# leggedrobotics/rayen

Measured on AMD Instinct MI355X. Metric: feasible projections/sec at k=64, 128 lin+4 quad+2 SOC; max violation, higher is better.
Workload: dtype f32

## Files before the change

rayen_amd/csrc/rayen_mfma_pair_wl.hip:

```cpp
#include "rayen_split_image.h"

#include <algorithm>
#include <cstdlib>
#include <mutex>
#include <type_traits>

namespace rayen {

namespace {
#ifndef RAYEN_WL_WAVES
#define RAYEN_WL_WAVES 16
#endif
#ifndef RAYEN_WL_NT
#define RAYEN_WL_NT 1
#endif
#ifndef RAYEN_WL_AHEAD
#define RAYEN_WL_AHEAD 0
#endif
constexpr int kWlWaves = RAYEN_WL_WAVES;
constexpr int kWlNT = RAYEN_WL_NT;
#ifndef RAYEN_WL_ABL
#define RAYEN_WL_ABL 0
#endif
#ifndef RAYEN_WL_HEAD
#define RAYEN_WL_HEAD 1
#endif
#ifndef RAYEN_WL_AUXR2
#define RAYEN_WL_AUXR2 16
#endif
template <int NKK, bool MAPPED = false> struct WlGeom { static constexpr int AUXR = NKK == 2 ? (MAPPED ? 8 : RAYEN_WL_AUXR2) : 32; };
#ifndef RAYEN_WL_SR
#define RAYEN_WL_SR 0
#endif
constexpr int wl_stage_rows(int nt) { return RAYEN_WL_SR ? RAYEN_WL_SR : (nt == 1 ? 16 : 32); }
constexpr int wl_region_bytes(int nkk, int nt) {
  return nt * (nkk == 2 ? WlGeom<2>::AUXR : WlGeom<1>::AUXR) * 128 > wl_stage_rows(nt) * 128 ? nt * (nkk == 2 ? WlGeom<2>::AUXR : WlGeom<1>::AUXR) * 128
                                                                                             : wl_stage_rows(nt) * 128;
}
__device__ __forceinline__ void wl_dma16(const char* gbase, const unsigned voff, const unsigned lds) {
  unsigned keep;
  uint64_t asm_base;
  asm volatile(RAYEN_ASM_BASE_COPY "s_mov_b32 %[k], m0\n\ts_mov_b32 m0, %[lds]\n\ts_nop 0\n\tglobal_load_lds_dwordx4 %[off], " RAYEN_ASM_BASE "\n\ts_mov_b32 m0, %[k]"
               : [k] "=&s"(keep), [b] "=&s"(asm_base)
               : [off] "v"(voff), [base] "s"(gbase), [lds] "s"(lds)
               : "memory");
}
#ifndef RAYEN_WL_SWAP
#define RAYEN_WL_SWAP 1
#endif
template <bool SWAP> __device__ __forceinline__ float wl_half_sum(const float x) {
  if constexpr (SWAP && RAYEN_WL_SWAP) {
    const unsigned u = __builtin_bit_cast(unsigned, x);
    const auto r = __builtin_amdgcn_permlane32_swap(u, u, false, false);
    return __builtin_bit_cast(float, (unsigned)r[0]) + __builtin_bit_cast(float, (unsigned)r[1]);
  } else {
    return x + xhalf(x);
  }
}
template <bool SWAP> __device__ __forceinline__ float wl_half_max(const float x) {
  if constexpr (SWAP && RAYEN_WL_SWAP) {
    const unsigned u = __builtin_bit_cast(unsigned, x);
    const auto r = __builtin_amdgcn_permlane32_swap(u, u, false, false);
    return fmaxf(__builtin_bit_cast(float, (unsigned)r[0]), __builtin_bit_cast(float, (unsigned)r[1]));
  } else {
    return fmaxf(x, xhalf(x));
  }
}
#ifndef RAYEN_WL_NANNV2
#define RAYEN_WL_NANNV2 1
#endif
__device__ __forceinline__ void wl_set_level(const int level) {
  if (level <= 0) __builtin_amdgcn_s_setprio(3);
  else if (level == 1) __builtin_amdgcn_s_setprio(2);
  else if (level == 2) __builtin_amdgcn_s_setprio(1);
  else __builtin_amdgcn_s_setprio(0);
}
constexpr int kWlStageRowsMapped = 8;
constexpr int wl_region_bytes_mapped(int nkk, int nt) {
  return nt * (nkk == 2 ? WlGeom<2, true>::AUXR : WlGeom<1, true>::AUXR) * 128 > kWlStageRowsMapped * 128
             ? nt * (nkk == 2 ? WlGeom<2, true>::AUXR : WlGeom<1, true>::AUXR) * 128
             : kWlStageRowsMapped * 128;
}
}

#ifdef RAYEN_WL_STAMPS
#ifndef RAYEN_WL_STAMP_ROUND
#define RAYEN_WL_STAMP_ROUND 1
#endif
__device__ unsigned long long wl_stamp_buf[2 * 40 * 4];
extern "C" int rayen_debug_wl_stamps(void* dst, size_t bytes) {
  return hipMemcpyFromSymbol(dst, HIP_SYMBOL(wl_stamp_buf), bytes < sizeof(wl_stamp_buf) ? bytes : sizeof(wl_stamp_buf)) == hipSuccess ? 0 : -1;
}
#define RAYEN_WL_STAMP(item, slot)                                                                              \
  do {                                                                                                          \
    if (stamp_on && lane == 0 && (item) < 40) wl_stamp_buf[((wave >> 2) * 40 + (item)) * 4 + (slot)] = __builtin_amdgcn_s_memtime(); \
  } while (0)
#else
#define RAYEN_WL_STAMP(item, slot) do { } while (0)
#endif
#ifdef RAYEN_WL_CLOCK
constexpr int kWlClockSlots = 10;
__device__ unsigned long long wl_clock_buf[16 * 16 * kWlClockSlots];
extern "C" int rayen_debug_wl_clock(void* dst, size_t bytes) {
  return hipMemcpyFromSymbol(dst, HIP_SYMBOL(wl_clock_buf), bytes < sizeof(wl_clock_buf) ? bytes : sizeof(wl_clock_buf)) == hipSuccess ? 0 : -1;
}
#define RAYEN_WL_CLOCK_AT(slot)                                               \
  do {                                                                        \
    if (probe) {                                                              \
      clock_at[2 * (slot) + 0] = __builtin_amdgcn_s_memtime();                \
      clock_at[2 * (slot) + 1] = __builtin_amdgcn_s_memrealtime();            \
    }                                                                         \
  } while (0)
#else
#define RAYEN_WL_CLOCK_AT(slot) do { } while (0)
#endif

template <int NKK, bool TRACK, int NT, int NW, int NKX = 0, bool SCREEN = false, bool DRAIN = false>
__global__ __launch_bounds__(NW * 64, 1) void mfma_pair_wl_kernel(
    const f16x8* __restrict__ Wh, const MItem* __restrict__ items, int n_items,
    const MPack* __restrict__ packs, const float* __restrict__ y0, int n_tiles, int n,
    const float* __restrict__ v, int64_t B, int64_t ldv, float* __restrict__ y, int64_t ldy,
    float* __restrict__ kappa_out, int32_t* __restrict__ active_out,
    int32_t* __restrict__ nan_flag, const float w_scale, const float w_inv,
    const f16x8* __restrict__ mimg, int n_in, float* __restrict__ v_out, int64_t ldvo,
    const WlScreen* __restrict__ scr, unsigned* __restrict__ scr_count, const int probe_on) {
  static_assert(!SCREEN || (NT == 1 && NKX == 0), "screening: one sample tile per wave, no mapper in front");
  static_assert(!DRAIN || NKX == 0, "progress-ordered priority: the instances without a mapper");
  constexpr int NS = NKK * 2, NCH = NS * 2, NQ = NKK * 4, AUXR = WlGeom<NKK, (NKX > 0)>::AUXR;
  constexpr int NSX = NKX * 2, NQX = NKX * 4, MCH = NKK * NSX * 2;
  constexpr bool SWAP = NKX == 0;
  constexpr bool NANNV2 = SCREEN && RAYEN_WL_NANNV2 != 0;
  extern __shared__ __attribute__((aligned(1024))) char wl_smem[];
  const int lane = threadIdx.x & 63;
  const int wave = __builtin_amdgcn_readfirstlane(threadIdx.x >> 6);
  const int col = lane & 31;
  const int hi = lane >> 5;
  char* const wimg = wl_smem;
  constexpr int REGION = NKX > 0 ? wl_region_bytes_mapped(NKK, NT) : wl_region_bytes(NKK, NT);
  constexpr int SR = NKX > 0 ? kWlStageRowsMapped : wl_stage_rows(NT);
  char* const mlds = wl_smem + (size_t)n_tiles * (NCH * 1024);
  char* const stage = mlds + MCH * 1024 + wave * REGION;
  float (*const aux_lds)[AUXR][32] = reinterpret_cast<float (*)[AUXR][32]>(stage);
  float* const y0_lds = reinterpret_cast<float*>(mlds + MCH * 1024 + NW * REGION);
  float* const bias_lds = y0_lds + NKK * 32;
  unsigned* const take_lds = reinterpret_cast<unsigned*>(bias_lds + (NKX > 0 ? NKK * 32 : 0));
  const int64_t n_groups = (B + NT * 32 - 1) / (NT * 32);
  const int64_t grp_stride = (int64_t)gridDim.x;
  int64_t grp = (int64_t)blockIdx.x + (int64_t)wave * grp_stride;
  bool bad = false;
  bool first_walk = true;
  unsigned skipped = 0;
#ifdef RAYEN_WL_STAMPS
  int stamp_round = 0;
  bool stamp_on = false;
#endif
#ifdef RAYEN_WL_CLOCK
  const bool probe = (blockIdx.x & 15) == 0 && (blockIdx.x >> 4) < 16;
  unsigned long long clock_at[8] = {0, 0, 0, 0, 0, 0, 0, 0};
  int clock_groups = 0;
  RAYEN_WL_CLOCK_AT(0);
#endif
  [[maybe_unused]] int drain_level = 0, drain_at = 0x7FFFFFFF;

  for (int i = threadIdx.x; i < NKK * 32; i += NW * 64) y0_lds[i] = y0[i];
  if (threadIdx.x == 0) *take_lds = NW;
  float gm_inv = 1.f;
  int gm_exp = 0;
  if constexpr (NKX > 0) {
    const float* tail = reinterpret_cast<const float*>(mimg + (size_t)MCH * 64);
    const float gm = tail[NKK * 32];
    gm_inv = tail[NKK * 32 + 1];
    gm_exp = (int)((__builtin_bit_cast(unsigned, gm) >> 23) & 255u) - 127;
    for (int i = threadIdx.x; i < NKK * 32; i += NW * 64) bias_lds[i] = tail[i] * gm;
  }
#if !(RAYEN_WL_HEAD & 1)
  {
    const int n_chunks = n_tiles * NCH;
    const char* src = reinterpret_cast<const char*>(Wh) + lane * 16;
#pragma unroll 4
    for (int c = wave; c < n_chunks; c += NW)
      *reinterpret_cast<u32x4*>(wimg + c * 1024 + lane * 16) = *reinterpret_cast<const u32x4*>(src + (size_t)c * 1024);
  }
#endif

  const __amdgpu_buffer_rsrc_t v_rsrc =
      __builtin_amdgcn_make_buffer_rsrc(const_cast<float*>(v), 0, (int)(unsigned)((uint64_t)B * (uint64_t)ldv * 4u), 0x00020000);
  const __amdgpu_buffer_rsrc_t y_rsrc =
      __builtin_amdgcn_make_buffer_rsrc(y, 0, (int)(unsigned)((uint64_t)B * (uint64_t)ldy * 4u), 0x00020000);
  const unsigned v_lane_off = (unsigned)col * (unsigned)ldv * 4u + 16u * (unsigned)hi;
  const unsigned y_lane_off = (unsigned)(lane >> 3) * (unsigned)ldy * 4u + 16u * (unsigned)((lane & 7) ^ ((lane >> 3) & 7));
  f32x4 vraw[NT][NQ];
  f32x4 xraw[NT][NKX > 0 ? NQX : 1];
  const bool ragged_n = n < NKK * 32;
  const bool ragged_in = NKX > 0 && n_in < NKX * 32;
  constexpr unsigned kNowhere = 0xFFFFFFF0u;
  auto request = [&](const int64_t g) {
    const unsigned goff = v_lane_off + (unsigned)g * (unsigned)(NT * 32) * (unsigned)ldv * 4u;
#pragma unroll
    for (int t = 0; t < NT; ++t) {
      if constexpr (NKX > 0) {
        if (__builtin_expect(ragged_in, 0)) {
          asm volatile("; ragged width" ::: "memory");
#pragma unroll
          for (int q = 0; q < NQX; ++q) {
            unsigned off = goff + (unsigned)t * 32u * (unsigned)ldv * 4u + 32u * q;
            off = (8 * q + 4 * hi < n_in) ? off : kNowhere;
            xraw[t][q] = __builtin_bit_cast(f32x4, __builtin_amdgcn_raw_buffer_load_b128(v_rsrc, off, 0, 0));
          }
        } else {
#pragma unroll
          for (int q = 0; q < NQX; ++q)
            xraw[t][q] = __builtin_bit_cast(f32x4, __builtin_amdgcn_raw_buffer_load_b128(
                v_rsrc, goff + (unsigned)t * 32u * (unsigned)ldv * 4u + 32u * q, 0, 0));
        }
      } else {
        if (__builtin_expect(ragged_n, 0)) {
          asm volatile("; ragged width" ::: "memory");
#pragma unroll
          for (int q = 0; q < NQ; ++q) {
            unsigned off = goff + (unsigned)t * 32u * (unsigned)ldv * 4u + 32u * q;
            off = (8 * q + 4 * hi < n) ? off : kNowhere;
            vraw[t][q] = __builtin_bit_cast(f32x4, __builtin_amdgcn_raw_buffer_load_b128(v_rsrc, off, 0, 0));
          }
        } else {
#pragma unroll
          for (int q = 0; q < NQ; ++q)
            vraw[t][q] = __builtin_bit_cast(f32x4, __builtin_amdgcn_raw_buffer_load_b128(
                v_rsrc, goff + (unsigned)t * 32u * (unsigned)ldv * 4u + 32u * q, 0, 0));
        }
      }
    }
  };
  float m_half[NT];
  auto half_max = [&]() {
#pragma unroll
    for (int t = 0; t < NT; ++t) {
      float m = 0.f;
      if constexpr (NKX > 0) {
#pragma unroll
        for (int q = 0; q < NQX; ++q)
#pragma unroll
          for (int c = 0; c < 4; ++c) m = fmaxf(m, __builtin_fabsf(xraw[t][q][c]));
      } else {
#pragma unroll
        for (int q = 0; q < NQ; ++q)
#pragma unroll
          for (int c = 0; c < 4; ++c) m = fmaxf(m, __builtin_fabsf(vraw[t][q][c]));
      }
      m_half[t] = m;
      asm volatile("" : "+v"(m_half[t]));
    }
  };
#pragma unroll
  for (int t = 0; t < NT; ++t) m_half[t] = 0.f;
  auto put_lines = [&](const f32x4 (&o)[4], const int h, const int t, const __amdgpu_buffer_rsrc_t rsrc, const unsigned goff,
                       const unsigned ld4, const int width, const bool ragged) {
#pragma unroll
    for (int part = 0; part < 32 / SR; ++part) {
      if (SR == 32 || (col / SR) == part) {
        char* slot = stage + (col % SR) * 128;
#pragma unroll
        for (int qq = 0; qq < 4; ++qq) *reinterpret_cast<f32x4*>(slot + (((2 * qq + hi) ^ (col & 7)) * 16)) = o[qq];
      }
      __builtin_amdgcn_wave_barrier();
#pragma unroll
      for (int i = 0; i < SR / 8; ++i) {
        const int r = 8 * i + (lane >> 3);
        const f32x4 x = *reinterpret_cast<const f32x4*>(stage + r * 128 + (lane & 7) * 16);
        unsigned off = goff + (unsigned)(t * 32 + part * SR + 8 * i) * ld4 + 128u * h;
        if (__builtin_expect(ragged, 0)) {
          asm volatile("; ragged width" ::: "memory");
          off = (32 * h + 4 * ((lane & 7) ^ ((lane >> 3) & 7)) < width) ? off : kNowhere;
        }
        if constexpr (RAYEN_WL_ABL & 2) { if (x[0] == 123.456f) __builtin_amdgcn_raw_buffer_store_b128(__builtin_bit_cast(u32x4, x), rsrc, off, 0, 0); }
        else if constexpr (RAYEN_WL_ABL & 8) __builtin_amdgcn_raw_buffer_store_b128(__builtin_bit_cast(u32x4, x), rsrc, off, 0, 0);
        else __builtin_amdgcn_raw_buffer_store_b128(__builtin_bit_cast(u32x4, x), rsrc, off, 0, 2);
      }
      __builtin_amdgcn_wave_barrier();
    }
  };
#if RAYEN_WL_HEAD
  {
    const int n_chunks = n_tiles * NCH;
    const unsigned img_at = __builtin_amdgcn_readfirstlane((unsigned)reinterpret_cast<uintptr_t>(wimg));
    const unsigned lane16 = lane * 16;
    if (RAYEN_WL_HEAD & 1)
      for (int c = wave; c < n_chunks; c += NW)
        wl_dma16(reinterpret_cast<const char*>(Wh) + (size_t)c * 1024, lane16, img_at + c * 1024);
    if constexpr (NKX > 0)
      for (int c = wave; c < MCH; c += NW)
        wl_dma16(reinterpret_cast<const char*>(mimg) + (size_t)c * 1024, lane16, img_at + (n_chunks + c) * 1024);
    if ((RAYEN_WL_HEAD & 2) && (grp + 1) * (NT * 32) <= B) {
      const char* gb = reinterpret_cast<const char*>(v + grp * (NT * 32) * ldv);
      const unsigned lds_at = __builtin_amdgcn_readfirstlane((unsigned)reinterpret_cast<uintptr_t>(stage));
#pragma unroll
      for (int t = 0; t < NT; ++t)
#pragma unroll
        for (int q = 0; q < NQ; ++q) wl_dma16(gb, v_lane_off + (unsigned)t * 32u * (unsigned)ldv * 4u + 32u * q, lds_at);
      asm volatile("s_waitcnt vmcnt(%0)" : : "n"(NT * NQ) : "memory");
    } else {
      asm volatile("s_waitcnt vmcnt(0)" ::: "memory");
    }
  }
#endif
  if (RAYEN_WL_AHEAD && grp < n_groups) {
    request(grp);
    half_max();
  }
  __syncthreads();

  while (grp < n_groups) {
    const int64_t s_base = grp * (NT * 32);
    int taken = 0;
    if (lane == 0) taken = (int)atomicAdd(take_lds, 1u);
    const int64_t next = (int64_t)blockIdx.x + (int64_t)__builtin_amdgcn_readfirstlane(taken) * grp_stride;
    bool live[NT];
#pragma unroll
    for (int t = 0; t < NT; ++t) live[t] = (s_base + t * 32 + col) < B;
    if constexpr (DRAIN) {
      wl_set_level(drain_level);
      drain_level = drain_level < 3 ? drain_level + 1 : 3;
      drain_at = next >= n_groups ? n_items / 3 : 0x7FFFFFFF;
    }
    if constexpr (!RAYEN_WL_AHEAD) {
      request(grp);
      half_max();
    }

#ifdef RAYEN_WL_STAMPS
    stamp_on = blockIdx.x == 0 && (wave == 0 || wave == 4) && stamp_round == RAYEN_WL_STAMP_ROUND;
    ++stamp_round;
    RAYEN_WL_STAMP(38, 0);
#endif
    f16x8 vb[NT][2][NS];
    float v_scl[NT], v_inv[NT];
    bool nan_row[NT];
    int sx_exp[NT];
    if constexpr (NKX > 0) {
      static_assert(NT == 1, "the mapped instances walk one sample tile per wave");
      static_assert((RAYEN_WL_HEAD & 1) != 0, "the mapper's image is copied by the LDS-DMA head");
      const unsigned vo_goff = (unsigned)(lane >> 3) * (unsigned)ldvo * 4u + 16u * (unsigned)((lane & 7) ^ ((lane >> 3) & 7)) +
                               (unsigned)s_base * (unsigned)ldvo * 4u;
      const __amdgpu_buffer_rsrc_t vo_rsrc =
          __builtin_amdgcn_make_buffer_rsrc(v_out, 0, (int)(unsigned)((uint64_t)B * (uint64_t)ldvo * 4u), 0x00020000);
#pragma unroll
      for (int t = 0; t < NT; ++t) {
        const float mx = fmaxf(m_half[t], xhalf(m_half[t]));
        float sx, sx_inv;
        pow2_scale(mx, sx, sx_inv, sx_exp[t]);
        f32x16 macc[NKK];
#pragma unroll
        for (int tp = 0; tp < NKK; ++tp)
#pragma unroll
          for (int a4 = 0; a4 < 4; ++a4) {
            const f32x4 b4 = *reinterpret_cast<const f32x4*>(&bias_lds[32 * tp + 8 * a4 + 4 * hi]);
#pragma unroll
            for (int c = 0; c < 4; ++c) macc[tp][4 * a4 + c] = b4[c] * sx;
          }
#pragma unroll
        for (int sxs = 0; sxs < NSX; ++sxs) {
          u32x4 w1, w2;
#pragma unroll
          for (int j = 0; j < 4; ++j) {
            const int q = 2 * sxs + (j >> 1), c = 2 * (j & 1);
            unsigned a, b;
            pair_split_lo(a, b, xraw[t][q][c], sx);
            pair_split_hi(a, b, xraw[t][q][c + 1], sx);
            w1[j] = a;
            w2[j] = b;
          }
          const f16x8 xb0 = __builtin_bit_cast(f16x8, w1), xb1 = __builtin_bit_cast(f16x8, w2);
#pragma unroll
          for (int tp = 0; tp < NKK; ++tp) {
            const char* ch = mlds + (size_t)((tp * NSX + sxs) * 2) * 1024 + lane * 16;
            const f16x8 a1 = __builtin_bit_cast(f16x8, *reinterpret_cast<const u32x4*>(ch));
            const f16x8 a2 = __builtin_bit_cast(f16x8, *reinterpret_cast<const u32x4*>(ch + 1024));
            macc[tp] = __builtin_amdgcn_mfma_f32_32x32x16_f16(a2, xb0, macc[tp], 0, 0, 0);
            macc[tp] = __builtin_amdgcn_mfma_f32_32x32x16_f16(a1, xb1, macc[tp], 0, 0, 0);
            macc[tp] = __builtin_amdgcn_mfma_f32_32x32x16_f16(a1, xb0, macc[tp], 0, 0, 0);
          }
        }
        if (v_out != nullptr) {
#pragma unroll
          for (int h = 0; h < NKK; ++h) {
            f32x4 o[4];
#pragma unroll
            for (int qq = 0; qq < 4; ++qq)
#pragma unroll
              for (int c = 0; c < 4; ++c) o[qq][c] = fmaf(macc[h][4 * qq + c] * gm_inv, sx_inv, 0.f);
            put_lines(o, h, t, vo_rsrc, vo_goff, (unsigned)ldvo * 4u, n, ragged_n);
          }
        }
        float m = 0.f;
#pragma unroll
        for (int q = 0; q < NQ; ++q)
#pragma unroll
          for (int c = 0; c < 4; ++c) {
            vraw[t][q][c] = macc[q >> 2][4 * (q & 3) + c];
            m = fmaxf(m, __builtin_fabsf(vraw[t][q][c]));
          }
        m_half[t] = m;
      }
    }
#pragma unroll
    for (int t = 0; t < NT; ++t) {
      const float m = wl_half_max<SWAP>(m_half[t]);
      float sv;
      int sv_exp;
      pow2_scale(m, sv, v_inv[t], sv_exp);
      v_scl[t] = sv;
      if constexpr (NKX > 0) {
        int e = sv_exp + gm_exp + sx_exp[t];
        e = e > 126 ? 126 : (e < -126 ? -126 : e);
        v_scl[t] = __builtin_bit_cast(float, (unsigned)(127 + e) << 23);
        v_inv[t] = __builtin_bit_cast(float, (unsigned)(127 - e) << 23);
      }
      f16x2 z = {(_Float16)0.f, (_Float16)0.f};
#pragma unroll
      for (int sp = 0; sp < NS; ++sp) {
        u32x4 w1, w2;
#pragma unroll
        for (int j = 0; j < 4; ++j) {
          const int q = 2 * sp + (j >> 1), c = 2 * (j & 1);
          unsigned a, b;
          pair_split_lo(a, b, vraw[t][q][c], sv);
          pair_split_hi(a, b, vraw[t][q][c + 1], sv);
          w1[j] = a;
          w2[j] = b;
          if constexpr (!NANNV2) pair_nan_fold(z, a);
        }
        vb[t][0][sp] = __builtin_bit_cast(f16x8, w1);
        vb[t][1][sp] = __builtin_bit_cast(f16x8, w2);
      }
      if constexpr (!NANNV2) nan_row[t] = pair_nan_seen(z);
    }
    float nv2 = 0.f;
    if constexpr (SCREEN) {
      float s0 = 0.f, s1 = 0.f;
#pragma unroll
      for (int q = 0; q < NQ; ++q)
#pragma unroll
        for (int c = 0; c < 4; c += 2) {
          const float x0 = vraw[0][q][c] * v_scl[0], x1 = vraw[0][q][c + 1] * v_scl[0];
          s0 = fmaf(x0, x0, s0);
          s1 = fmaf(x1, x1, s1);
        }
      nv2 = wl_half_sum<SWAP>(s0 + s1);
      if constexpr (NANNV2) nan_row[0] = !(nv2 < __builtin_inff());
    }
    __builtin_amdgcn_sched_barrier(0);
    if (RAYEN_WL_AHEAD && next < n_groups && !(RAYEN_WL_ABL & 1)) request(next);
    __builtin_amdgcn_sched_barrier(0);

    float kap[NT], part[NT];
    int acode[NT];
#pragma unroll
    for (int t = 0; t < NT; ++t) { kap[t] = 0.f; part[t] = 0.f; acode[t] = -1; }
    {
      f32x16 acc[NT];
      const f32x16 zero = {0.f, 0.f, 0.f, 0.f, 0.f, 0.f, 0.f, 0.f, 0.f, 0.f, 0.f, 0.f, 0.f, 0.f, 0.f, 0.f};
      const int ts_first = items[0].tile_shape;
      int ts_next = ts_first;
      u32x4 abuf[NCH];
      auto fetch = [&](const int ts_of) {
        const char* tb = wimg + (size_t)(ts_of & 0xFFFFFF) * (NCH * 1024) + lane * 16;
        if constexpr (NS == 4) {
          const int shape = __builtin_amdgcn_readfirstlane((ts_of >> 24) & 3);
          if (shape != MS_HALF_B) {
#pragma unroll
            for (int c = 0; c < 4; ++c) abuf[c] = *reinterpret_cast<const u32x4*>(tb + c * 1024);
          }
          if (shape != MS_HALF_A) {
#pragma unroll
            for (int c = 4; c < 8; ++c) abuf[c] = *reinterpret_cast<const u32x4*>(tb + c * 1024);
          }
        } else {
#pragma unroll
          for (int c = 0; c < NCH; ++c) abuf[c] = *reinterpret_cast<const u32x4*>(tb + c * 1024);
        }
      };
      if (first_walk) {
        fetch(ts_first);
        first_walk = false;
      }
      const int n_walk = n_items - ((RAYEN_WL_ABL & 64) ? 4 : 0);
      for (int it = 0; it < n_walk; ++it) {
        RAYEN_WL_STAMP(it, 0);
        if constexpr (DRAIN) {
          if (it >= drain_at) {
            wl_set_level(drain_level);
            drain_level = drain_level < 3 ? drain_level + 1 : 3;
            drain_at = drain_at < 2 * (n_items / 3) ? 2 * (n_items / 3) : 0x7FFFFFFF;
          }
        }
#ifdef RAYEN_WL_CLOCK
        if (it == 0 && clock_groups == 0) RAYEN_WL_CLOCK_AT(1);
#endif
        const int ts = ts_next;
        auto burst = [&](auto S0, auto S1) {
          constexpr int s0 = decltype(S0)::value, s1 = decltype(S1)::value;
#pragma unroll
          for (int sp = s0; sp < s1; ++sp) {
            const f16x8 a1 = __builtin_bit_cast(f16x8, abuf[2 * sp + 0]), a2 = __builtin_bit_cast(f16x8, abuf[2 * sp + 1]);
#pragma unroll
            for (int t = 0; t < NT; ++t)
              acc[t] = __builtin_amdgcn_mfma_f32_32x32x16_f16(a2, vb[t][0][sp], sp == s0 ? zero : acc[t], 0, 0, 0);
#pragma unroll
            for (int t = 0; t < NT; ++t) acc[t] = __builtin_amdgcn_mfma_f32_32x32x16_f16(a1, vb[t][1][sp], acc[t], 0, 0, 0);
          }
#pragma unroll
          for (int sp = s0; sp < s1; ++sp) {
            const f16x8 a1 = __builtin_bit_cast(f16x8, abuf[2 * sp + 0]);
#pragma unroll
            for (int t = 0; t < NT; ++t) acc[t] = __builtin_amdgcn_mfma_f32_32x32x16_f16(a1, vb[t][0][sp], acc[t], 0, 0, 0);
          }
        };
        __builtin_amdgcn_sched_barrier(0);
        if constexpr (RAYEN_WL_ABL & 32) {
#pragma unroll
          for (int t = 0; t < NT; ++t)
#pragma unroll
            for (int g = 0; g < 16; ++g) acc[t][g] = __builtin_bit_cast(float, __builtin_bit_cast(u32x4, vb[t][0][g & 3])[g >> 2]);
        } else if constexpr (NS == 4) {
          const int shape = __builtin_amdgcn_readfirstlane((ts >> 24) & 3);
          if (shape == MS_FULL) burst(std::integral_constant<int, 0>{}, std::integral_constant<int, 4>{});
          else if (shape == MS_HALF_A) burst(std::integral_constant<int, 0>{}, std::integral_constant<int, 2>{});
          else burst(std::integral_constant<int, 2>{}, std::integral_constant<int, 4>{});
        } else {
          burst(std::integral_constant<int, 0>{}, std::integral_constant<int, NS>{});
        }
        __builtin_amdgcn_sched_barrier(0);
        const MItem item = items[it];
        WlScreen sc_next;
        if constexpr (SCREEN) sc_next = scr[it + 1];
        ts_next = (it + 1 < n_walk) ? item.qbegin : ts_first;
        if constexpr (!(RAYEN_WL_ABL & 32)) fetch(ts_next);
        RAYEN_WL_STAMP(it, 1);
        __builtin_amdgcn_sched_barrier(0);
        if constexpr (RAYEN_WL_ABL & 16) {
#pragma unroll
          for (int t = 0; t < NT; ++t) kap[t] = fmaxf(kap[t], acc[t][0]);
          continue;
        }

        if (item.type == MI_LIN) {
          const int lin_code = (item.seg << 20) + item.row0 + 4 * hi;
#pragma unroll
          for (int t = 0; t < NT; ++t) {
            if (TRACK) {
#pragma unroll
              for (int g = 0; g < 16; ++g)
                if (acc[t][g] > kap[t]) {
                  kap[t] = acc[t][g];
                  acode[t] = lin_code + ((g & 3) + 8 * (g >> 2));
                }
            } else {
#pragma unroll
              for (int g = 0; g < 16; ++g) kap[t] = fmaxf(kap[t], acc[t][g]);
            }
          }
        } else if (item.type == MI_QFAC || item.type == MI_SOC) {
#pragma unroll
          for (int t = 0; t < NT; ++t) {
            float s0 = (item.flags & MF_FIRST) ? 0.f : part[t], s1 = 0.f;
#pragma unroll
            for (int g = 0; g < 16; g += 2) {
              s0 = fmaf(acc[t][g], acc[t][g], s0);
              s1 = fmaf(acc[t][g + 1], acc[t][g + 1], s1);
            }
            part[t] = s0 + s1;
          }
          if (item.flags & MF_LAST) {
#pragma unroll
            for (int t = 0; t < NT; ++t) {
              const float total = wl_half_sum<SWAP>(part[t]);
              const float a0 = aux_lds[t][item.aux][col];
              float kc;
              if (item.type != MI_SOC) {
                kc = (a0 + __builtin_amdgcn_sqrtf(fmaxf(total, 0.f))) * item.seg_inv;
              } else {
                kc = pair_soc_candidate(a0, aux_lds[t][item.aux + 1][col], total, w_inv * item.seg_inv, v_inv[t], item.f0,
                                        item.f1, v_scl[t], w_scale);
              }
              if (kc > kap[t]) { kap[t] = kc; acode[t] = item.seg << 20; }
            }
          }
        } else if (item.type == MI_AUX) {
#pragma unroll
          for (int t = 0; t < NT; ++t)
#pragma unroll
            for (int g = 0; g < AUXR / 2; ++g) aux_lds[t][(g & 3) + 8 * (g >> 2) + 4 * hi][col] = acc[t][g];
          __builtin_amdgcn_wave_barrier();
        } else if (item.type == MI_PACK) {
          const MPack pk = packs[item.aux];
#pragma unroll
          for (int a = 0; a < 4; ++a) {
            const int slot = hi ? pk.aux[a][1] : pk.aux[a][0];
            const int sid = hi ? pk.seg[a][1] : pk.seg[a][0];
            const bool pair = (item.row0 >> a) & 1;
#pragma unroll
            for (int t = 0; t < NT; ++t) {
              float qs = acc[t][4 * a] * acc[t][4 * a];
#pragma unroll
              for (int c = 1; c < 4; ++c) qs = fmaf(acc[t][4 * a + c], acc[t][4 * a + c], qs);
              if (pair) qs = wl_half_sum<SWAP>(qs);
              const float kc = (aux_lds[t][slot & (AUXR - 1)][col] + __builtin_amdgcn_sqrtf(qs)) * (hi ? pk.inv[a][1] : pk.inv[a][0]);
              if (sid >= 0 && kc > kap[t]) { kap[t] = kc; acode[t] = sid << 20; }
            }
          }
        }
        RAYEN_WL_STAMP(it, 2);
        if constexpr (SCREEN) {
          if (sc_next.cnst > 0.f || sc_next.cabs > 0.f) {
            WlScreen s = sc_next;
            int nx = it + 1, ts_to = ts_next;
            int ts_held = ts_next;
            auto kmax_now = [&] { return wl_half_max<SWAP>(kap[0]); };
            const bool nv_ok = nv2 < __builtin_inff();
            const bool probe_row = (nv2 >= 67108864.f) || (nv2 == 0.f);
            for (;;) {
              bool skip = false;
              if (s.cnst > 0.f) {
                const float tb = s.cnst * nv2;
                const float a0 = aux_lds[0][s.aux][col];
                float ub;
                if (!(s.span >> 16)) {
                  ub = (a0 + __builtin_amdgcn_sqrtf(fmaxf(tb, 0.f))) * s.seg_inv;
                } else {
                  ub = pair_soc_candidate(a0, aux_lds[0][s.aux + 1][col], tb, w_inv * s.seg_inv, v_inv[0], s.f0, s.f1, v_scl[0], w_scale);
                }
                const bool below = (ub < kmax_now()) && nv_ok;
                skip = __ballot(live[0] && !below) == 0;
              }
              if (!skip && probe_on != 0 && s.cabs > 0.f) {
                const int span = s.span & 0xFFFF;
                int ts_j = ts_to;
                for (int j = 0; j < span; ++j) {
                  const char* tb = wimg + (size_t)(ts_j & 0xFFFFFF) * (NCH * 1024) + lane * 16;
                  const int shape = NS == 4 ? __builtin_amdgcn_readfirstlane((ts_j >> 24) & 3) : MS_FULL;
                  auto lead = [&](auto S0, auto S1) {
                    constexpr int s0 = decltype(S0)::value, s1 = decltype(S1)::value;
                    if (ts_j != ts_held) {
#pragma unroll
                      for (int sp = s0; sp < s1; ++sp) abuf[2 * sp] = *reinterpret_cast<const u32x4*>(tb + (2 * sp) * 1024);
                      ts_held = -2;
                    }
#pragma unroll
                    for (int sp = s0; sp < s1; ++sp)
                      acc[0] = __builtin_amdgcn_mfma_f32_32x32x16_f16(__builtin_bit_cast(f16x8, abuf[2 * sp]), vb[0][0][sp],
                                                                      sp == s0 ? zero : acc[0], 0, 0, 0);
                  };
                  if constexpr (NS == 4) {
                    if (shape == MS_FULL) lead(std::integral_constant<int, 0>{}, std::integral_constant<int, 4>{});
                    else if (shape == MS_HALF_A) lead(std::integral_constant<int, 0>{}, std::integral_constant<int, 2>{});
                    else lead(std::integral_constant<int, 2>{}, std::integral_constant<int, 4>{});
                  } else {
                    lead(std::integral_constant<int, 0>{}, std::integral_constant<int, NS>{});
                  }
                  if (j + 1 < span) ts_j = items[nx + j].qbegin;
                  float s0 = j == 0 ? 0.f : part[0], s1 = 0.f;
#pragma unroll
                  for (int g = 0; g < 16; g += 2) {
                    s0 = fmaf(acc[0][g], acc[0][g], s0);
                    s1 = fmaf(acc[0][g + 1], acc[0][g + 1], s1);
                  }
                  part[0] = s0 + s1;
                }
                const float total = wl_half_sum<SWAP>(part[0]);
                const float r = __builtin_amdgcn_sqrtf(fmaxf(total, 0.f)) + __builtin_amdgcn_sqrtf(s.cabs * nv2);
                const float tb = (r * r) * 1.000244140625f;
                const float a0 = aux_lds[0][s.aux][col];
                float ub;
                if (!(s.span >> 16)) {
                  ub = (a0 + __builtin_amdgcn_sqrtf(fmaxf(tb, 0.f))) * s.seg_inv;
                } else {
                  ub = pair_soc_candidate(a0, aux_lds[0][s.aux + 1][col], tb, w_inv * s.seg_inv, v_inv[0], s.f0, s.f1, v_scl[0], w_scale);
                }
                const bool below = (ub < kmax_now()) && nv_ok && probe_row;
                skip = __ballot(live[0] && !below) == 0;
              }
              if (!skip) break;
              nx += s.span & 0xFFFF;
              ts_to = s.ts_after;
              skipped += (lane == s.seg) ? 1u : 0u;
              if (ts_to < 0) break;
              s = scr[nx];
              if (!(s.cnst > 0.f) && !(s.cabs > 0.f)) break;
            }
            if (nx != it + 1) {
              ts_next = ts_to < 0 ? ts_first : ts_to;
              it = nx - 1;
            }
            if (ts_held != ts_next) fetch(ts_next);
          }
        }
      }
    }
    RAYEN_WL_STAMP(38, 1);

    float knat[NT], scale[NT];
#pragma unroll
    for (int t = 0; t < NT; ++t) {
      if (TRACK || !SWAP) {
        const float other = xhalf(kap[t]);
        if (TRACK) {
          const int ocode = __shfl_xor(acode[t], 32);
          if (other > kap[t] || (other == kap[t] && hi == 1)) acode[t] = ocode;
        }
        kap[t] = fmaxf(kap[t], other);
      } else {
        kap[t] = wl_half_max<SWAP>(kap[t]);
      }
      knat[t] = (kap[t] * w_inv) * v_inv[t];
      scale[t] = v_inv[t] * (1.0f / fmaxf(1.0f, knat[t]));
    }
    if (hi == 0) {
#pragma unroll
      for (int t = 0; t < NT; ++t) {
        if (!live[t]) continue;
        const int64_t s = s_base + t * 32 + col;
        if (kappa_out) kappa_out[s] = knat[t];
        if (TRACK) { active_out[2 * s] = acode[t] >> 20; active_out[2 * s + 1] = acode[t] < 0 ? 0 : (acode[t] & 0xFFFFF); }
      }
    }

    __builtin_amdgcn_sched_barrier(0);
    if constexpr (RAYEN_WL_AHEAD) half_max();
    __builtin_amdgcn_sched_barrier(0);

    const unsigned y_goff = y_lane_off + (unsigned)s_base * (unsigned)ldy * 4u;
#pragma unroll
    for (int t = 0; t < NT; ++t) {
      float one = 1.0f;
      asm volatile("" : "+v"(one));
#pragma unroll
      for (int h = 0; h < NKK; ++h) {
        f32x4 o[4];
#pragma unroll
        for (int qq = 0; qq < 4; ++qq) {
          const int q = 4 * h + qq;
          const f32x4 o4 = *reinterpret_cast<const f32x4*>(&y0_lds[8 * q + 4 * hi]);
#pragma unroll
          for (int c = 0; c < 4; ++c) {
            const int i = (q & 1) * 4 + c;
            const unsigned w1 = __builtin_bit_cast(u32x4, vb[t][0][q >> 1])[i >> 1], w2 = __builtin_bit_cast(u32x4, vb[t][1][q >> 1])[i >> 1];
            const float val = (i & 1) ? pair_rebuild_hi(w1, w2, one) : pair_rebuild_lo(w1, w2, one);
            o[qq][c] = fmaf(val, scale[t], o4[c]);
          }
        }
        put_lines(o, h, t, y_rsrc, y_goff, (unsigned)ldy * 4u, n, ragged_n);
      }
      bad |= live[t] && nan_row[t];
    }
    RAYEN_WL_STAMP(38, 2);
#ifdef RAYEN_WL_CLOCK
    if (clock_groups == 0) RAYEN_WL_CLOCK_AT(2);
    ++clock_groups;
#endif
    grp = next;
  }
  if (nan_flag && bad) atomicOr(nan_flag, 1);
  if constexpr (SCREEN) {
    if (scr_count != nullptr && skipped != 0) atomicAdd(scr_count + lane, skipped);
  }
#ifdef RAYEN_WL_CLOCK
  RAYEN_WL_CLOCK_AT(3);
  if (probe && lane == 0) {
    unsigned long long* const rec = wl_clock_buf + ((blockIdx.x >> 4) * 16 + (wave & 15)) * kWlClockSlots;
#pragma unroll
    for (int i = 0; i < 8; ++i) rec[i] = clock_at[i];
    rec[8] = __builtin_amdgcn_s_getreg(63492);
    rec[9] = (unsigned long long)clock_groups;
  }
#endif
}

static int pair_wl_lds_bytes_mapped(const PairImage* img, int nkx) {
  return img->n_tiles * (img->nkk * 4 * 1024) + img->nkk * (nkx * 2) * 2 * 1024 + kWlWaves * wl_region_bytes_mapped(img->nkk, 1) +
         2 * img->nkk * 128 + 16;
}
static int pair_wl_lds_bytes(const PairImage* img) {
  return img->n_tiles * (img->nkk * 4 * 1024) + kWlWaves * wl_region_bytes(img->nkk, kWlNT) + img->nkk * 128 + 16;
}

bool mfma_pair_wl_serves(const RayenPack* p, const PairImage* img, const float* v, int64_t B, int64_t ldv,
                         const float* y, int64_t ldy) {
  if (img == nullptr || img->nkk < 1 || img->nkk > 2 || img->n_tiles <= 0 || !img->wl_ready) return false;
  if (!img->identity || p->k != p->n || p->n > img->nkk * 32 || p->n <= (img->nkk - 1) * 32 || (p->n % 4) != 0) return false;
  if (ldv < p->n || ldy < p->n) return false;
  if ((ldv % 4) != 0 || (ldy % 4) != 0) return false;
  if (ldv > (1 << 22) || ldy > (1 << 22)) return false;
  if (!base_aligned16(v) || !base_aligned16(y)) return false;
  if (img->nkk == 2 && img->aux_rows > WlGeom<2>::AUXR) return false;
  if (pair_wl_lds_bytes(img) > 160 * 1024) return false;
  const int64_t n_groups = (B + kWlNT * 32 - 1) / (kWlNT * 32);
  static const int64_t min_groups_env = [] { const char* e = getenv("RAYEN_WL_MIN_GROUPS"); return e ? atoll(e) : 1ll; }();
  return n_groups >= min_groups_env;
}

static thread_local unsigned* wl_gate_counters = nullptr;
static thread_local int wl_gate_mode = 1;

static void wl_screen_gate(const RayenPack* p, PairImage* img, const bool gate) {
  constexpr int kProbe = 4096;
  constexpr double kMinShare = 0.25;
  constexpr double kMinProbeShare = 0.5;
  const int n = p->n;
  auto drop = [&] {
    (void)hipFree(img->wl_screen);
    img->wl_screen = nullptr;
    img->host_screen.clear();
    if (img->wl_items) (void)hipFree(img->wl_items);
    img->wl_items = nullptr;
    img->wl_host_items.clear();
  };
  std::vector<float> dirs((size_t)kProbe * n);
  uint64_t state = 0x9E3779B97F4A7C15ull;
  for (float& x : dirs) {
    state = state * 6364136223846793005ull + 1442695040888963407ull;
    x = (float)((double)(state >> 11) / (double)(1ull << 53) * 2.0 - 1.0);
  }
  float *dv = nullptr, *dy = nullptr;
  unsigned* dc = nullptr;
  int32_t* da = nullptr;
  unsigned counts_s[64] = {0}, counts_b[64] = {0};
  std::vector<int32_t> act((size_t)2 * kProbe, -1);
  auto launch = [&](const int mode, int32_t* active) {
    wl_gate_counters = dc;
    wl_gate_mode = mode;
    const bool fine = mfma_pair_wl_forward(p, img, dv, kProbe, n, dy, n, nullptr, active, nullptr, nullptr) == RAYEN_OK;
    wl_gate_counters = nullptr;
    wl_gate_mode = 1;
    return fine && hipStreamSynchronize(nullptr) == hipSuccess;
  };
  bool ok = hipMalloc(&dv, dirs.size() * sizeof(float)) == hipSuccess && hipMalloc(&dy, dirs.size() * sizeof(float)) == hipSuccess &&
            hipMalloc(&dc, sizeof(counts_s)) == hipSuccess && hipMalloc(&da, act.size() * sizeof(int32_t)) == hipSuccess &&
            hipMemcpy(dv, dirs.data(), dirs.size() * sizeof(float), hipMemcpyHostToDevice) == hipSuccess &&
            hipMemset(dc, 0, sizeof(counts_s)) == hipSuccess;
  ok = ok && launch(0, da) && hipMemcpy(act.data(), da, act.size() * sizeof(int32_t), hipMemcpyDeviceToHost) == hipSuccess;
  if (ok) {
    std::vector<uint64_t> hits(p->segs.size(), 0);
    for (int r = 0; r < kProbe; ++r) {
      const int32_t sg = act[(size_t)2 * r];
      if (sg >= 0 && (size_t)sg < hits.size()) ++hits[sg];
    }
    std::vector<MItem> own = img->host_items;
    std::vector<WlScreen> tab = img->host_screen;
    if (pair_wl_reorder(own, tab, hits)) {
      ok = upload_to_device(own, &img->wl_items, &img->bytes) &&
           hipMemcpy(img->wl_screen, tab.data(), tab.size() * sizeof(WlScreen), hipMemcpyHostToDevice) == hipSuccess;
      if (ok) {
        img->wl_host_items.swap(own);
        img->host_screen.swap(tab);
      }
    }
  }
  if (ok && gate) {
    ok = launch(2, nullptr) && hipMemcpy(counts_s, dc, sizeof(counts_s), hipMemcpyDeviceToHost) == hipSuccess &&
         hipMemset(dc, 0, sizeof(counts_s)) == hipSuccess && launch(1, nullptr) &&
         hipMemcpy(counts_b, dc, sizeof(counts_b), hipMemcpyDeviceToHost) == hipSuccess;
  }
  if (dv) (void)hipFree(dv);
  if (dy) (void)hipFree(dy);
  if (dc) (void)hipFree(dc);
  if (da) (void)hipFree(da);
  if (!ok) { drop(); return; }
  if (!gate) return;
  bool any = false, changed = false;
  const double groups = kProbe / 32;
  for (WlScreen& s : img->host_screen) {
    if (!(s.cnst > 0.f) && !(s.cabs > 0.f)) continue;
    const double by_bound = counts_s[s.seg], by_both = counts_b[s.seg] > counts_s[s.seg] ? counts_b[s.seg] : counts_s[s.seg];
    const bool keep_bound = s.cnst > 0.f && by_bound >= kMinShare * groups;
    const double left = keep_bound ? groups - by_bound : groups, by_probe = keep_bound ? by_both - by_bound : by_both;
    const bool keep_probe = s.cabs > 0.f && left > 0.0 && by_probe >= kMinProbeShare * left;
    if (!keep_bound && s.cnst > 0.f) { s.cnst = 0.f; changed = true; }
    if (!keep_probe && s.cabs > 0.f) { s.cabs = 0.f; changed = true; }
    any = any || keep_bound || keep_probe;
  }
  if (!any) { drop(); return; }
  if (changed && hipMemcpy(img->wl_screen, img->host_screen.data(), img->host_screen.size() * sizeof(WlScreen), hipMemcpyHostToDevice) != hipSuccess)
    drop();
}

int mfma_pair_wl_prepare(const RayenPack* p, PairImage* img) {
  if (img == nullptr || img->nkk < 1 || img->nkk > 2 || img->n_tiles <= 0 || !img->identity) return RAYEN_OK;
  const int lds = pair_wl_lds_bytes(img);
  if (lds > 160 * 1024) return RAYEN_OK;
  static std::mutex mu;
  static int promised = 0;
  std::lock_guard<std::mutex> hold(mu);
  promised = std::max(promised, lds);
  const int ask = promised;
  bool ok = true;
  auto want = [&](auto kern) {
    ok = ok && hipFuncSetAttribute(reinterpret_cast<const void*>(kern), hipFuncAttributeMaxDynamicSharedMemorySize, ask) == hipSuccess;
  };
  want(mfma_pair_wl_kernel<1, false, kWlNT, kWlWaves>); want(mfma_pair_wl_kernel<1, true, kWlNT, kWlWaves>);
  want(mfma_pair_wl_kernel<2, false, kWlNT, kWlWaves>); want(mfma_pair_wl_kernel<2, true, kWlNT, kWlWaves>);
  if constexpr (kWlNT == 1) {
    want(mfma_pair_wl_kernel<1, false, 1, kWlWaves, 0, true>); want(mfma_pair_wl_kernel<1, true, 1, kWlWaves, 0, true>);
    want(mfma_pair_wl_kernel<2, false, 1, kWlWaves, 0, true>); want(mfma_pair_wl_kernel<2, true, 1, kWlWaves, 0, true>);
  }
  want(mfma_pair_wl_kernel<1, false, kWlNT, kWlWaves, 0, false, true>); want(mfma_pair_wl_kernel<1, true, kWlNT, kWlWaves, 0, false, true>);
  want(mfma_pair_wl_kernel<2, false, kWlNT, kWlWaves, 0, false, true>); want(mfma_pair_wl_kernel<2, true, kWlNT, kWlWaves, 0, false, true>);
  if constexpr (kWlNT == 1) {
    want(mfma_pair_wl_kernel<1, false, 1, kWlWaves, 0, true, true>); want(mfma_pair_wl_kernel<1, true, 1, kWlWaves, 0, true, true>);
    want(mfma_pair_wl_kernel<2, false, 1, kWlWaves, 0, true, true>); want(mfma_pair_wl_kernel<2, true, 1, kWlWaves, 0, true, true>);
  }
  if (!ok) return RAYEN_E_LAUNCH;
  img->wl_ready = true;
  const char* gate_env = getenv("RAYEN_PAIR_SCREEN_GATE");
  if (kWlNT == 1 && img->wl_screen != nullptr) wl_screen_gate(p, img, !(gate_env != nullptr && gate_env[0] == '0'));
  const int lds_m = pair_wl_lds_bytes_mapped(img, img->nkk);
  if (kWlNT == 1 && lds_m <= 160 * 1024) {
    static int promised_m = 0;
    promised_m = std::max(promised_m, lds_m);
    const int ask_m = promised_m;
    auto want_m = [&](auto kern) {
      ok = ok && hipFuncSetAttribute(reinterpret_cast<const void*>(kern), hipFuncAttributeMaxDynamicSharedMemorySize, ask_m) == hipSuccess;
    };
    want_m(mfma_pair_wl_kernel<1, false, 1, kWlWaves, 1>); want_m(mfma_pair_wl_kernel<1, true, 1, kWlWaves, 1>);
    want_m(mfma_pair_wl_kernel<2, false, 1, kWlWaves, 1>); want_m(mfma_pair_wl_kernel<2, true, 1, kWlWaves, 1>);
    want_m(mfma_pair_wl_kernel<2, false, 1, kWlWaves, 2>); want_m(mfma_pair_wl_kernel<2, true, 1, kWlWaves, 2>);
    if (!ok) return RAYEN_E_LAUNCH;
    img->wl_mapped_ready = true;
  }
  return RAYEN_OK;
}

bool mfma_pair_wl_serves_mapped(const RayenPack* p, const PairImage* img, const float* x, int64_t B, int64_t ldx, int in_dim,
                                const float* v_out, int64_t ldvo, const float* y, int64_t ldy) {
  if (kWlNT != 1 || img == nullptr || img->nkk < 1 || img->nkk > 2 || img->n_tiles <= 0 || !img->wl_mapped_ready) return false;
  if (!img->identity || p->k != p->n || p->n > img->nkk * 32 || p->n <= (img->nkk - 1) * 32 || (p->n % 4) != 0) return false;
  if (in_dim < 4 || in_dim > img->nkk * 32 || (in_dim % 4) != 0 || ldx < in_dim || ldy < p->n) return false;
  if ((ldx % 4) != 0 || (ldy % 4) != 0 || ldx > (1 << 22) || ldy > (1 << 22)) return false;
  if (!base_aligned16(x) || !base_aligned16(y)) return false;
  if (v_out != nullptr && ((ldvo % 4) != 0 || ldvo < p->n || ldvo > (1 << 22) || !base_aligned16(v_out))) return false;
  if (img->nkk == 2 && img->aux_rows > WlGeom<2, true>::AUXR) return false;
  if (pair_wl_lds_bytes_mapped(img, (in_dim + 31) / 32) > 160 * 1024) return false;
  static const int64_t min_groups_env = [] { const char* e = getenv("RAYEN_WL_MIN_GROUPS"); return e ? atoll(e) : 1ll; }();
  return B >= 1 && (B + 31) / 32 >= min_groups_env;
}

int mfma_pair_wl_forward_mapped(const RayenPack* p, const PairImage* img, const float* x, int64_t B, int64_t ldx, int in_dim,
                                const void* image, float* v_out, int64_t ldvo, float* y, int64_t ldy, float* kappa,
                                int32_t* active, int32_t* nan_flag, hipStream_t stream) {
  if (B == 0) return RAYEN_OK;
  if (image == nullptr || !mfma_pair_wl_serves_mapped(p, img, x, B, ldx, in_dim, v_out, ldvo, y, ldy)) return RAYEN_E_UNSUPPORTED;
  const int nkx = (in_dim + 31) / 32;
  const int64_t cus = launch_simds(img->n_simd) / 4;
  const int lds = pair_wl_lds_bytes_mapped(img, nkx);
  const int64_t ld_max = std::max<int64_t>(std::max(std::max(ldx, ldy), v_out ? ldvo : 1), 1);
  const int64_t rows_max = (((int64_t)0xFFFFFFFFll / (ld_max * 4)) - 64) / 32 * 32;
  for (int64_t r0 = 0; r0 < B; r0 += rows_max) {
    const int64_t Bc = std::min(B - r0, rows_max);
    const int64_t n_groups = (Bc + 31) / 32;
    const unsigned grid = (unsigned)std::min<int64_t>(cus, n_groups);
    const float* xc = x + r0 * ldx;
    float* yc = y + r0 * ldy;
    float* voc = v_out ? v_out + r0 * ldvo : nullptr;
    float* kc = kappa ? kappa + r0 : nullptr;
    int32_t* ac = active ? active + 2 * r0 : nullptr;
    auto go = [&](auto kern) {
      hipLaunchKernelGGL(kern, dim3(grid), dim3(kWlWaves * 64), lds, stream, static_cast<const f16x8*>(img->Wh), img->items,
                         img->n_items, img->packs, img->y0, img->n_tiles, p->n, xc, Bc, ldx, yc, ldy, kc, ac, nan_flag,
                         img->w_scale, img->w_inv, static_cast<const f16x8*>(image), in_dim, voc, ldvo,
                         static_cast<const WlScreen*>(nullptr), static_cast<unsigned*>(nullptr), 0);
    };
    if (img->nkk == 1) {
      if (active != nullptr) go(mfma_pair_wl_kernel<1, true, 1, kWlWaves, 1>);
      else go(mfma_pair_wl_kernel<1, false, 1, kWlWaves, 1>);
    } else if (nkx == 1) {
      if (active != nullptr) go(mfma_pair_wl_kernel<2, true, 1, kWlWaves, 1>);
      else go(mfma_pair_wl_kernel<2, false, 1, kWlWaves, 1>);
    } else {
      if (active != nullptr) go(mfma_pair_wl_kernel<2, true, 1, kWlWaves, 2>);
      else go(mfma_pair_wl_kernel<2, false, 1, kWlWaves, 2>);
    }
  }
  return hipGetLastError() == hipSuccess ? RAYEN_OK : RAYEN_E_LAUNCH;
}

int mfma_pair_wl_forward(const RayenPack* p, const PairImage* img, const float* v, int64_t B, int64_t ldv,
                         float* y, int64_t ldy, float* kappa, int32_t* active, int32_t* nan_flag,
                         hipStream_t stream) {
  if (B == 0) return RAYEN_OK;
  if (!mfma_pair_wl_serves(p, img, v, B, ldv, y, ldy)) return RAYEN_E_UNSUPPORTED;
  const int64_t cus = launch_simds(img->n_simd) / 4;
  const int lds = pair_wl_lds_bytes(img);
  const int64_t ld_max = std::max<int64_t>(std::max(ldv, ldy), 1);
  const int64_t rows_max = (((int64_t)0xFFFFFFFFll / (ld_max * 4)) - 64) / (kWlNT * 32) * (kWlNT * 32);
  const int mode = wl_gate_counters != nullptr ? wl_gate_mode : pair_screen_cell().load(std::memory_order_relaxed);
  const bool screen = kWlNT == 1 && img->wl_screen != nullptr && mode != 0;
  const int probe_on = mode == 1 ? 1 : 0;
  unsigned* const counters = wl_gate_counters != nullptr ? wl_gate_counters : pair_screen_counters_cell().load(std::memory_order_relaxed);
  const bool drain_on = wl_gate_counters == nullptr && pair_drain_cell().load(std::memory_order_relaxed) != 0;
  const MItem* const items = img->wl_items != nullptr ? img->wl_items : img->items;
  for (int64_t r0 = 0; r0 < B; r0 += rows_max) {
    const int64_t Bc = std::min(B - r0, rows_max);
    const int64_t n_groups = (Bc + kWlNT * 32 - 1) / (kWlNT * 32);
    const unsigned grid = (unsigned)std::min<int64_t>(cus, n_groups);
    const float* vc = v + r0 * ldv;
    float* yc = y + r0 * ldy;
    float* kc = kappa ? kappa + r0 : nullptr;
    int32_t* ac = active ? active + 2 * r0 : nullptr;
    auto go = [&](auto kern) {
      hipLaunchKernelGGL(kern, dim3(grid), dim3(kWlWaves * 64), lds, stream, static_cast<const f16x8*>(img->Wh), items,
                         img->n_items, img->packs, img->y0, img->n_tiles, p->n, vc, Bc, ldv, yc, ldy, kc, ac, nan_flag,
                         img->w_scale, img->w_inv, static_cast<const f16x8*>(nullptr), 0, static_cast<float*>(nullptr), (int64_t)0,
                         screen ? img->wl_screen : nullptr, screen ? counters : nullptr, probe_on);
    };
    auto pick = [&](auto drain) {
      constexpr bool D = decltype(drain)::value;
      if constexpr (kWlNT == 1) {
        if (screen) {
          if (img->nkk == 1) {
            if (active != nullptr) go(mfma_pair_wl_kernel<1, true, 1, kWlWaves, 0, true, D>);
            else go(mfma_pair_wl_kernel<1, false, 1, kWlWaves, 0, true, D>);
          } else {
            if (active != nullptr) go(mfma_pair_wl_kernel<2, true, 1, kWlWaves, 0, true, D>);
            else go(mfma_pair_wl_kernel<2, false, 1, kWlWaves, 0, true, D>);
          }
          return;
        }
      }
      if (img->nkk == 1) {
        if (active != nullptr) go(mfma_pair_wl_kernel<1, true, kWlNT, kWlWaves, 0, false, D>);
        else go(mfma_pair_wl_kernel<1, false, kWlNT, kWlWaves, 0, false, D>);
      } else {
        if (active != nullptr) go(mfma_pair_wl_kernel<2, true, kWlNT, kWlWaves, 0, false, D>);
        else go(mfma_pair_wl_kernel<2, false, kWlNT, kWlWaves, 0, false, D>);
      }
    };
    if (drain_on) pick(std::true_type{});
    else pick(std::false_type{});
  }
  return hipGetLastError() == hipSuccess ? RAYEN_OK : RAYEN_E_LAUNCH;
}

}
```

Before: 6.736 billion.

## Prefetch first sample rows during head and issue next group's loads at loop tail

```diff
diff --git a/rayen_amd/csrc/rayen_mfma_pair_wl.hip b/rayen_amd/csrc/rayen_mfma_pair_wl.hip
--- a/rayen_amd/csrc/rayen_mfma_pair_wl.hip
+++ b/rayen_amd/csrc/rayen_mfma_pair_wl.hip
@@ -23,7 +23,13 @@
 #define RAYEN_WL_ABL 0
 #endif
 #ifndef RAYEN_WL_HEAD
-#define RAYEN_WL_HEAD 1
+#define RAYEN_WL_HEAD 5
+#endif
+#ifndef RAYEN_WL_EARLY
+#define RAYEN_WL_EARLY 2
+#endif
+#ifndef RAYEN_WL_KMAX_ONCE
+#define RAYEN_WL_KMAX_ONCE 1
 #endif
 #ifndef RAYEN_WL_AUXR2
 #define RAYEN_WL_AUXR2 16
@@ -130,6 +136,7 @@
   constexpr int NSX = NKX * 2, NQX = NKX * 4, MCH = NKK * NSX * 2;
   constexpr bool SWAP = NKX == 0;
   constexpr bool NANNV2 = SCREEN && RAYEN_WL_NANNV2 != 0;
+  constexpr bool ROWS_FIRST = (RAYEN_WL_HEAD & 4) != 0 && (RAYEN_WL_HEAD & 2) == 0 && NKX == 0 && RAYEN_WL_AHEAD == 0;
   extern __shared__ __attribute__((aligned(1024))) char wl_smem[];
   const int lane = threadIdx.x & 63;
   const int wave = __builtin_amdgcn_readfirstlane(threadIdx.x >> 6);
@@ -194,7 +201,8 @@
   const bool ragged_n = n < NKK * 32;
   const bool ragged_in = NKX > 0 && n_in < NKX * 32;
   constexpr unsigned kNowhere = 0xFFFFFFF0u;
-  auto request = [&](const int64_t g) {
+  auto request = [&](const int64_t g, auto one_copy) {
+    constexpr bool ONE = decltype(one_copy)::value;
     const unsigned goff = v_lane_off + (unsigned)g * (unsigned)(NT * 32) * (unsigned)ldv * 4u;
 #pragma unroll
     for (int t = 0; t < NT; ++t) {
@@ -214,7 +222,14 @@
                 v_rsrc, goff + (unsigned)t * 32u * (unsigned)ldv * 4u + 32u * q, 0, 0));
         }
       } else {
-        if (__builtin_expect(ragged_n, 0)) {
+        if constexpr (ONE) {
+#pragma unroll
+          for (int q = 0; q < NQ; ++q) {
+            unsigned off = goff + (unsigned)t * 32u * (unsigned)ldv * 4u + 32u * q;
+            off = (8 * q + 4 * hi < n) ? off : kNowhere;
+            vraw[t][q] = __builtin_bit_cast(f32x4, __builtin_amdgcn_raw_buffer_load_b128(v_rsrc, off, 0, 0));
+          }
+        } else if (__builtin_expect(ragged_n, 0)) {
           asm volatile("; ragged width" ::: "memory");
 #pragma unroll
           for (int q = 0; q < NQ; ++q) {
@@ -298,16 +313,22 @@
 #pragma unroll
         for (int q = 0; q < NQ; ++q) wl_dma16(gb, v_lane_off + (unsigned)t * 32u * (unsigned)ldv * 4u + 32u * q, lds_at);
       asm volatile("s_waitcnt vmcnt(%0)" : : "n"(NT * NQ) : "memory");
+    } else if (ROWS_FIRST && wave < RAYEN_WL_EARLY && grp < n_groups) {
+      request(grp, std::true_type{});
+      asm volatile("s_waitcnt vmcnt(%0)" : : "n"(NT * NQ) : "memory");
     } else {
       asm volatile("s_waitcnt vmcnt(0)" ::: "memory");
     }
   }
 #endif
   if (RAYEN_WL_AHEAD && grp < n_groups) {
-    request(grp);
+    request(grp, std::false_type{});
     half_max();
   }
   __syncthreads();
+  if constexpr (ROWS_FIRST) {
+    if (wave >= RAYEN_WL_EARLY && grp < n_groups) request(grp, std::true_type{});
+  }
 
   while (grp < n_groups) {
     const int64_t s_base = grp * (NT * 32);
@@ -323,7 +344,7 @@
       drain_at = next >= n_groups ? n_items / 3 : 0x7FFFFFFF;
     }
     if constexpr (!RAYEN_WL_AHEAD) {
-      request(grp);
+      if constexpr (!ROWS_FIRST) request(grp, std::false_type{});
       half_max();
     }
 
@@ -449,7 +470,7 @@
       if constexpr (NANNV2) nan_row[0] = !(nv2 < __builtin_inff());
     }
     __builtin_amdgcn_sched_barrier(0);
-    if (RAYEN_WL_AHEAD && next < n_groups && !(RAYEN_WL_ABL & 1)) request(next);
+    if (RAYEN_WL_AHEAD && next < n_groups && !(RAYEN_WL_ABL & 1)) request(next, std::false_type{});
     __builtin_amdgcn_sched_barrier(0);
 
     float kap[NT], part[NT];
@@ -614,8 +635,9 @@
           if (sc_next.cnst > 0.f || sc_next.cabs > 0.f) {
             WlScreen s = sc_next;
             int nx = it + 1, ts_to = ts_next;
-            int ts_held = ts_next;
-            auto kmax_now = [&] { return wl_half_max<SWAP>(kap[0]); };
+            const int ts_held = ts_next;
+            [[maybe_unused]] const float kmax_held = wl_half_max<SWAP>(kap[0]);
+            auto kmax_now = [&] { return RAYEN_WL_KMAX_ONCE ? kmax_held : wl_half_max<SWAP>(kap[0]); };
             const bool nv_ok = nv2 < __builtin_inff();
             const bool probe_row = (nv2 >= 67108864.f) || (nv2 == 0.f);
             for (;;) {
@@ -640,14 +662,12 @@
                   const int shape = NS == 4 ? __builtin_amdgcn_readfirstlane((ts_j >> 24) & 3) : MS_FULL;
                   auto lead = [&](auto S0, auto S1) {
                     constexpr int s0 = decltype(S0)::value, s1 = decltype(S1)::value;
-                    if (ts_j != ts_held) {
-#pragma unroll
-                      for (int sp = s0; sp < s1; ++sp) abuf[2 * sp] = *reinterpret_cast<const u32x4*>(tb + (2 * sp) * 1024);
-                      ts_held = -2;
-                    }
+                    u32x4 pa[NS];
+#pragma unroll
+                    for (int sp = s0; sp < s1; ++sp) pa[sp] = *reinterpret_cast<const u32x4*>(tb + (2 * sp) * 1024);
 #pragma unroll
                     for (int sp = s0; sp < s1; ++sp)
-                      acc[0] = __builtin_amdgcn_mfma_f32_32x32x16_f16(__builtin_bit_cast(f16x8, abuf[2 * sp]), vb[0][0][sp],
+                      acc[0] = __builtin_amdgcn_mfma_f32_32x32x16_f16(__builtin_bit_cast(f16x8, pa[sp]), vb[0][0][sp],
                                                                       sp == s0 ? zero : acc[0], 0, 0, 0);
                   };
                   if constexpr (NS == 4) {
@@ -757,6 +777,10 @@
     if (clock_groups == 0) RAYEN_WL_CLOCK_AT(2);
     ++clock_groups;
 #endif
+    if constexpr (ROWS_FIRST) {
+      __builtin_amdgcn_sched_barrier(0);
+      if (next < n_groups) request(next, std::false_type{});
+    }
     grp = next;
   }
   if (nan_flag && bad) atomicOr(nan_flag, 1);
```

New measurement: 6.838 billion, median of 6. 1.5% higher.
